# dayae1204/WeCLIP-ViT-CoMer

Measured on AMD Instinct MI355X. Metric: images/sec (train fwd+bwd) ViT-B/16 512x512 VOC, higher is better.
Workload: dtype f16 MFMA operands / f32 accumulate, f32 residual+softmax+LN, PAR f32 arithmetic on 16-bit fixed-point affinities (precision=fast); 1 GPU; WeCLIP VOC full train step (the reference's model: frozen CLIP ViT-B/16 + adapters + decoder + GradCAM/affinity/PAR pseudo-labels), batch 16/GPU at 512x512, K=2 classes/image (BASELINE configs[2] without the ViT-CoMer inserts, for which the reference has no code); global_batch=16, parallelism=dp1

## Files before the change

### weclip-vit-comer_amd/csrc/attention.hip

```cpp
#include "common.h"
#include <stdlib.h>

typedef _Float16 f16x8 __attribute__((ext_vector_type(8)));
typedef _Float16 f16x4 __attribute__((ext_vector_type(4)));
typedef _Float16 f16x2 __attribute__((ext_vector_type(2)));
typedef float f32x16 __attribute__((ext_vector_type(16)));

#define NEG_BIG (-1.0e30f)

template <int DH, int NT>
__device__ __forceinline__ void attn_row_body(const __half* __restrict__ qkv, __half* __restrict__ out,
                                              float* __restrict__ out32, float* __restrict__ lse, int L, int H,
                                              int E, int q, int h, int b, float* lds) {
    constexpr int NCH = DH / 8;
    constexpr int NPT = NT / NCH;
    float* sc = lds;
    float* red = lds + ((L + 3) & ~3);
    float (*part)[DH] = reinterpret_cast<float (*)[DH]>(red + 16);
    const int tid = threadIdx.x;
    const long ldq = 3L * E;
    const __half* base = qkv + (long)b * L * ldq + (long)h * DH;
    f16x8 qv[NCH];
#pragma unroll
    for (int c = 0; c < NCH; ++c) qv[c] = *reinterpret_cast<const f16x8*>(base + (long)q * ldq + c * 8);
    float mx = NEG_BIG;
    for (int key = tid; key < L; key += NT) {
        const __half* kr = base + E + (long)key * ldq;
        float s = 0.f;
#pragma unroll
        for (int c = 0; c < NCH; ++c) {
            const f16x8 kv = *reinterpret_cast<const f16x8*>(kr + c * 8);
#pragma unroll
            for (int j = 0; j < 8; ++j) s = fmaf((float)qv[c][j], (float)kv[j], s);
        }
        sc[key] = s;
        mx = fmaxf(mx, s);
    }
    mx = block_max(mx, red);
    float sum = 0.f;
    for (int key = tid; key < L; key += NT) {
        const float pr = __builtin_amdgcn_exp2f(sc[key] - mx);
        sum += pr;
        sc[key] = (float)(_Float16)pr;
    }
    sum = block_sum(sum, red);
    const int ch = tid % NCH, pt = tid / NCH;
    float o[8];
#pragma unroll
    for (int j = 0; j < 8; ++j) o[j] = 0.f;
    const __half* vcol = base + 2 * E + ch * 8;
    int key = pt;
    for (; key + 3 * NPT < L; key += 4 * NPT) {
        f16x8 v[4];
#pragma unroll
        for (int u = 0; u < 4; ++u) v[u] = *reinterpret_cast<const f16x8*>(vcol + (long)(key + u * NPT) * ldq);
#pragma unroll
        for (int u = 0; u < 4; ++u) {
            const float pr = sc[key + u * NPT];
#pragma unroll
            for (int j = 0; j < 8; ++j) o[j] = fmaf(pr, (float)v[u][j], o[j]);
        }
    }
    for (; key < L; key += NPT) {
        const f16x8 v = *reinterpret_cast<const f16x8*>(vcol + (long)key * ldq);
        const float pr = sc[key];
#pragma unroll
        for (int j = 0; j < 8; ++j) o[j] = fmaf(pr, (float)v[j], o[j]);
    }
#pragma unroll
    for (int j = 0; j < 8; ++j) part[pt][ch * 8 + j] = o[j];
    __syncthreads();
    if (tid < DH) {
        float v = 0.f;
        for (int k = 0; k < NPT; ++k) v += part[k][tid];
        v /= sum;
        const long oi = ((long)b * L + q) * E + (long)h * DH + tid;
        out[oi] = __float2half(v);
        if (out32) out32[oi] = v;
        if (tid == 0) lse[((long)b * H + h) * L + q] = mx + log2f(sum);
    }
}

#define ATT_EDGE_MAX 8
template <int DH, int NW>
__global__ __launch_bounds__(NW * 64, 4) void attn_fwd_kernel(const __half* __restrict__ qkv,
                                                        __half* __restrict__ out,
                                                        float* __restrict__ out32,
                                                        float* __restrict__ lse, int L, int H,
                                                        int E, int q_origin, int nqb, int Bn, int k_origin) {
    constexpr int NT = NW * 64;
    constexpr int KS = DH / 16;
    constexpr int DT = DH / 32;
    constexpr int KROW = DH * 2 + 16;
    constexpr int VROW = DH * 2;
    constexpr int KBUF = 64 * KROW, VBUF = 64 * VROW;
    constexpr int KCH = DH / 8;
    constexpr int TCH = 64 * KCH;
    constexpr int NKC = (TCH + NT - 1) / NT;
    constexpr int NVC = NKC;
    extern __shared__ __attribute__((aligned(16))) char smem[];

    const int tid = threadIdx.x, lane = tid & 63, wave = tid >> 6;
    const int hh = lane >> 5, l31 = lane & 31;
    const int per_img = nqb * H;
    const int main_blocks = per_img * ((Bn + 7) / 8 * 8);
    if ((int)blockIdx.x >= main_blocks) {
        const int e = blockIdx.x - main_blocks;
        const int hb = e / q_origin;
        attn_row_body<DH, NT>(qkv, out, out32, lse, L, H, E, e - hb * q_origin, hb % H, hb / H, reinterpret_cast<float*>(smem));
        return;
    }
    const int slot = blockIdx.x >> 3;
    const int b = (slot / per_img) * 8 + (blockIdx.x & 7);
    if (b >= Bn) return;
    const int rem = slot - (slot / per_img) * per_img;
    const int h = rem / nqb, qb = rem - h * nqb;
    const int qrow = q_origin + qb * (NW * 32) + wave * 32 + l31;
    const int qr = qrow < L ? qrow : L - 1;
    const long ldq = 3L * E;
    const __half* base = qkv + (long)b * L * ldq + (long)h * DH;

    f16x8 qf[KS];
#pragma unroll
    for (int s = 0; s < KS; ++s)
        qf[s] = *reinterpret_cast<const f16x8*>(base + (long)qr * ldq + 16 * s + 8 * hh);

    u32x4 rk[NKC], rv[NVC];
#define VSWZ(key_) (DH == 64 ? ((((key_) >> 1) & 1) << 2) : 0)
    int vaddr[2];
    {
        const int gi = (lane >> 4) & 1, q4 = (lane >> 2) & 3, p4 = lane & 3;
#pragma unroll
        for (int r = 0; r < 2; ++r) {
            const int key = 8 * r + 4 * hh + q4;
            vaddr[r] = key * VROW + (((2 * gi + (p4 >> 1)) ^ VSWZ(key)) << 4) + 8 * (p4 & 1);
        }
    }
    typedef short s16x4 __attribute__((__vector_size__(4 * sizeof(short))));
    typedef __attribute__((address_space(3))) s16x4* tr_ptr;
#undef GLOAD
#define GLOAD(t_) \
    { \
        const int t__ = (t_); \
        _Pragma("unroll") \
        for (int i = 0; i < NKC; ++i) { \
            const int c = (NKC * NT == TCH) ? tid + NT * i : (tid + NT * i) % TCH;    \
            int key = k_origin + t__ * 64 + c / KCH; \
            if (key > L - 1) key = L - 1; \
            rk[i] = *reinterpret_cast<const u32x4*>(base + E + (long)key * ldq + (c % KCH) * 8); \
        } \
        _Pragma("unroll") \
        for (int i = 0; i < NVC; ++i) { \
            const int c = (NKC * NT == TCH) ? tid + NT * i : (tid + NT * i) % TCH; \
            int key = k_origin + t__ * 64 + c / KCH; \
            if (key > L - 1) key = L - 1; \
            rv[i] = *reinterpret_cast<const u32x4*>(base + 2 * E + (long)key * ldq + (c % KCH) * 8); \
        } \
    }
#undef LSTORE
#define LSTORE(buf_) \
    { \
        const int buf__ = (buf_); \
        char* kb = smem + buf__ * (KBUF + VBUF); \
        char* vb = kb + KBUF; \
        _Pragma("unroll") \
        for (int i = 0; i < NKC; ++i) { \
            const int c = tid + NT * i; \
            if (c < TCH) *reinterpret_cast<u32x4*>(kb + (c / KCH) * KROW + (c % KCH) * 16) = rk[i]; \
        } \
        _Pragma("unroll") \
        for (int i = 0; i < NVC; ++i) { \
            const int c = tid + NT * i; \
            const int key__ = c / KCH; \
            if (c < TCH) *reinterpret_cast<u32x4*>(vb + key__ * VROW + (((c % KCH) ^ VSWZ(key__)) << 4)) = rv[i]; \
        } \
    }

    f32x16 o[DT];
#pragma unroll
    for (int d = 0; d < DT; ++d)
#pragma unroll
        for (int r = 0; r < 16; ++r) o[d][r] = 0.f;
    float m = NEG_BIG, lsum = 0.f;

    const int nt = (L - k_origin + 63) / 64;
    GLOAD(0);
    LSTORE(0);
    __syncthreads();
    for (int t = 0; t < nt; ++t) {
        const int buf = t & 1;
        if (t + 1 < nt) GLOAD(t + 1);
        const char* kb = smem + buf * (KBUF + VBUF);
        const char* vb = kb + KBUF;
        f32x16 s[2];
#pragma unroll
        for (int r = 0; r < 16; ++r) { s[0][r] = 0.f; s[1][r] = 0.f; }
#pragma unroll
        for (int ks = 0; ks < KS; ++ks) {
            const f16x8 a0 = *reinterpret_cast<const f16x8*>(kb + l31 * KROW + ks * 32 + hh * 16);
            const f16x8 a1 = *reinterpret_cast<const f16x8*>(kb + (32 + l31) * KROW + ks * 32 + hh * 16);
            s[0] = __builtin_amdgcn_mfma_f32_32x32x16_f16(a0, qf[ks], s[0], 0, 0, 0);
            s[1] = __builtin_amdgcn_mfma_f32_32x32x16_f16(a1, qf[ks], s[1], 0, 0, 0);
        }
        if (t == nt - 1) {
#pragma unroll
            for (int ti = 0; ti < 2; ++ti)
#pragma unroll
                for (int r = 0; r < 16; ++r) {
                    const int key = k_origin + t * 64 + ti * 32 + (r & 3) + 8 * (r >> 2) + 4 * hh;
                    if (key >= L) s[ti][r] = NEG_BIG;
                }
        }
        float mx = s[0][0];
#pragma unroll
        for (int r = 1; r < 16; ++r) mx = fmaxf(mx, s[0][r]);
#pragma unroll
        for (int r = 0; r < 16; ++r) mx = fmaxf(mx, s[1][r]);
        mx = fmaxf(mx, __shfl_xor(mx, 32, 64));
        const float mn = fmaxf(m, mx);
        const float alpha = __builtin_amdgcn_exp2f(m - mn);
        m = mn;
        lsum *= alpha;
#pragma unroll
        for (int d = 0; d < DT; ++d) o[d] *= alpha;
        typedef float f32x2 __attribute__((ext_vector_type(2)));
        const f32x2 nm = {-m, -m};
        f32x2 ps2 = {0.f, 0.f};
#pragma unroll
        for (int ti = 0; ti < 2; ++ti)
#pragma unroll
            for (int r = 0; r < 16; r += 2) {
                f32x2 e = {s[ti][r], s[ti][r + 1]};
                e += nm;
                f32x2 p;
                p[0] = __builtin_amdgcn_exp2f(e[0]);
                p[1] = __builtin_amdgcn_exp2f(e[1]);
                s[ti][r] = p[0];
                s[ti][r + 1] = p[1];
                ps2 += p;
            }
        lsum += ps2[0] + ps2[1];
#pragma unroll
        for (int s2 = 0; s2 < 4; ++s2) {
            f16x8 pb;
#pragma unroll
            for (int j = 0; j < 8; ++j) pb[j] = (_Float16)s[s2 >> 1][(s2 & 1) * 8 + j];
#pragma unroll
            for (int d = 0; d < DT; ++d) {
                const char* vr = vb + s2 * 16 * VROW;
                const f16x8 va = __builtin_bit_cast(f16x8, __builtin_shufflevector(
                    __builtin_amdgcn_ds_read_tr16_b64_v4i16((tr_ptr)(vr + (vaddr[0] ^ (d << 6)))),
                    __builtin_amdgcn_ds_read_tr16_b64_v4i16((tr_ptr)(vr + (vaddr[1] ^ (d << 6)))), 0, 1, 2, 3, 4, 5, 6, 7));
                o[d] = __builtin_amdgcn_mfma_f32_32x32x16_f16(va, pb, o[d], 0, 0, 0);
            }
        }
        if (t + 1 < nt) LSTORE(buf ^ 1);
        __syncthreads();
    }
    if constexpr (NW == 8)
    for (int kx = 0; kx < k_origin; ++kx) {
        const __half* krow = base + E + (long)kx * ldq;
        float sdot = 0.f;
#pragma unroll
        for (int ks = 0; ks < KS; ++ks) {
            const f16x8 kv = *reinterpret_cast<const f16x8*>(krow + 16 * ks + 8 * hh);
#pragma unroll
            for (int j = 0; j < 8; ++j) sdot = fmaf((float)qf[ks][j], (float)kv[j], sdot);
        }
        sdot += __shfl_xor(sdot, 32, 64);
        const float mn = fmaxf(m, sdot);
        const float alpha = __builtin_amdgcn_exp2f(m - mn);
        const float pr = __builtin_amdgcn_exp2f(sdot - mn);
        m = mn;
        lsum = lsum * alpha + (hh == 0 ? pr : 0.f);
        const float p16 = (float)(_Float16)pr;
        const __half* vrow = base + 2 * E + (long)kx * ldq;
#pragma unroll
        for (int d = 0; d < DT; ++d)
#pragma unroll
            for (int g = 0; g < 4; ++g) {
                const f16x4 vv = *reinterpret_cast<const f16x4*>(vrow + d * 32 + 8 * g + 4 * hh);
#pragma unroll
                for (int k = 0; k < 4; ++k) o[d][g * 4 + k] = fmaf(p16, (float)vv[k], o[d][g * 4 + k] * alpha);
            }
    }
    const float ltot = lsum + __shfl_xor(lsum, 32, 64);
    const float inv = 1.0f / ltot;
#ifdef WC_NO_OSTAGE
    constexpr bool OSTAGE = false;
#else
    constexpr bool OSTAGE = NW == 8;
#endif
    if constexpr (OSTAGE) {
        constexpr int OPITCH = DH * 2 + 8;
        constexpr int CPR = DH / 8;
        char* stg = smem + wave * (32 * OPITCH);
    #pragma unroll
        for (int d = 0; d < DT; ++d)
    #pragma unroll
            for (int g = 0; g < 4; ++g) {
                __half hv[4];
    #pragma unroll
                for (int k = 0; k < 4; ++k) hv[k] = __float2half(o[d][g * 4 + k] * inv);
                *reinterpret_cast<uint2*>(stg + l31 * OPITCH + (d * 32 + 8 * g + 4 * hh) * 2) = *reinterpret_cast<uint2*>(hv);
            }
        asm volatile("s_waitcnt lgkmcnt(0)" ::: "memory");
        __builtin_amdgcn_wave_barrier();
        const int qw0 = q_origin + qb * (NW * 32) + wave * 32;
    #pragma unroll
        for (int i = 0; i < 32 * CPR / 64; ++i) {
            const int r = i * (64 / CPR) + lane / CPR, ch = lane % CPR;
            if (qw0 + r < L) {
                const uint2 lo2 = *reinterpret_cast<const uint2*>(stg + r * OPITCH + ch * 16);
                const uint2 hi2 = *reinterpret_cast<const uint2*>(stg + r * OPITCH + ch * 16 + 8);
                u32x4 v = {lo2.x, lo2.y, hi2.x, hi2.y};
                *reinterpret_cast<u32x4*>(out + ((long)b * L + qw0 + r) * E + (long)h * DH + ch * 8) = v;
            }
        }
    } else if (qrow < L) {
        __half* orow = out + ((long)b * L + qrow) * E + (long)h * DH;
#pragma unroll
        for (int d = 0; d < DT; ++d)
#pragma unroll
            for (int g = 0; g < 4; ++g) {
                __half hv[4];
#pragma unroll
                for (int k = 0; k < 4; ++k) hv[k] = __float2half(o[d][g * 4 + k] * inv);
                *reinterpret_cast<uint2*>(orow + d * 32 + 8 * g + 4 * hh) = *reinterpret_cast<uint2*>(hv);
            }
    }
    if (qrow < L) {
        if (out32) {
#pragma unroll
            for (int d = 0; d < DT; ++d)
#pragma unroll
                for (int g = 0; g < 4; ++g)
                    *reinterpret_cast<float4*>(out32 + ((long)b * L + qrow) * E + (long)h * DH + d * 32 + 8 * g + 4 * hh) =
                        make_float4(o[d][g * 4] * inv, o[d][g * 4 + 1] * inv, o[d][g * 4 + 2] * inv, o[d][g * 4 + 3] * inv);
        }
        if (hh == 0) lse[((long)b * H + h) * L + qrow] = m + log2f(ltot);
    }
}

template <int DH, int R>
__global__ __launch_bounds__(256, 2) void attn_mean_kernel(const __half* __restrict__ qkv,
                                                         const float* __restrict__ lse,
                                                         float* __restrict__ mean, int L, int H, int E, int origin,
                                                         int nt, int Bn) {
    constexpr int KS = DH / 16;
    constexpr int ROW = DH * 2 + 16;
    constexpr int TB = 128 * ROW;
    constexpr int CH = DH / 8;
    constexpr int NC = 128 * CH / 256;
    extern __shared__ __attribute__((aligned(16))) char smem[];
    constexpr int EDGE = 2 * TB + 512;
    constexpr int BUF = EDGE + (R > 0 ? 2 * R * DH * 2 + 32 : 0);

    const int tid = threadIdx.x, lane = tid & 63, wave = tid >> 6;
    const int hh = lane >> 5, l31 = lane & 31;
    const int wr = wave >> 1, wc = wave & 1;
    const int slot = blockIdx.x >> 3;
    const int b = (slot / (nt * nt)) * 8 + (blockIdx.x & 7);
    if (b >= Bn) return;
    const int rem = slot - (slot / (nt * nt)) * (nt * nt);
    const int k0 = origin + (rem % nt) * 128, q0 = origin + (rem / nt) * 128;
    const long ldq = 3L * E;
    const __half* base = qkv + (long)b * L * ldq;

    const bool edge_wg = R > 0 && (q0 == origin || k0 == origin);
    const bool edge_row = R > 0 && q0 == origin && tid < 128;
    const bool edge_col = R > 0 && k0 == origin && tid >= 128;
    const int e_which = tid / (origin * CH > 0 ? origin * CH : 1);
    const int e_rem = tid - e_which * origin * CH;
    const __half* e_src = base + (long)(e_rem / CH) * ldq + (e_which ? E : 0) + (e_rem % CH) * 8;
    const int e_dst = EDGE + (e_which * R * CH + e_rem) * 16;
    u32x4 rq[NC], rk[NC], re = {0u, 0u, 0u, 0u};
    float rl = 0.f;
#undef GLOAD
#define GLOAD(h_) \
    { \
        const int h__ = (h_); \
        _Pragma("unroll") \
        for (int i = 0; i < NC; ++i) { \
            const int c = tid + 256 * i; \
            int qr = q0 + c / CH, kr = k0 + c / CH; \
            if (qr > L - 1) qr = L - 1; \
            if (kr > L - 1) kr = L - 1; \
            rq[i] = *reinterpret_cast<const u32x4*>(base + (long)qr * ldq + h__ * DH + (c % CH) * 8); \
            rk[i] = *reinterpret_cast<const u32x4*>(base + (long)kr * ldq + E + h__ * DH + (c % CH) * 8); \
        } \
        if (tid < 128) { \
            int qr = q0 + tid; \
            if (qr > L - 1) qr = L - 1; \
            rl = lse[((long)b * H + h__) * L + qr]; \
        } \
        if constexpr (R > 0) \
            if (edge_wg) { \
                if (e_which < 2) re = *reinterpret_cast<const u32x4*>(e_src + h__ * DH); \
                if (tid >= 128 && tid < 128 + origin) rl = lse[((long)b * H + h__) * L + tid - 128]; \
            } \
    }
#undef LSTORE
#define LSTORE(buf_) \
    { \
        const int buf__ = (buf_); \
        char* qb = smem + buf__ * BUF; \
        _Pragma("unroll") \
        for (int i = 0; i < NC; ++i) { \
            const int c = tid + 256 * i; \
            *reinterpret_cast<u32x4*>(qb + (c / CH) * ROW + (c % CH) * 16) = rq[i]; \
            *reinterpret_cast<u32x4*>(qb + TB + (c / CH) * ROW + (c % CH) * 16) = rk[i]; \
        } \
        if (tid < 128) reinterpret_cast<float*>(qb + 2 * TB)[tid] = rl; \
        if constexpr (R > 0) \
            if (edge_wg) { \
                if (e_which < 2) *reinterpret_cast<u32x4*>(qb + e_dst) = re; \
                if (tid >= 128 && tid < 128 + origin) reinterpret_cast<float*>(qb + EDGE + 2 * R * DH * 2)[tid - 128] = rl; \
            } \
    }

    f32x16 acc[2][2];
#pragma unroll
    for (int i = 0; i < 2; ++i)
#pragma unroll
        for (int j = 0; j < 2; ++j)
#pragma unroll
            for (int r = 0; r < 16; ++r) acc[i][j][r] = 0.f;
    f16x8 b_aug;
#pragma unroll
    for (int j = 0; j < 8; ++j) b_aug[j] = (_Float16)((hh == 0 && j < 2) ? 1.0f : 0.0f);
    float eacc[R > 0 ? R : 1];
#pragma unroll
    for (int e = 0; e < (R > 0 ? R : 1); ++e) eacc[e] = 0.f;

    GLOAD(0);
    LSTORE(0);
    __syncthreads();
    for (int h = 0; h < H; ++h) {
        const int buf = h & 1;
        if (h + 1 < H) GLOAD(h + 1);
        const char* qb = smem + buf * BUF;
        const float* ls = reinterpret_cast<const float*>(qb + 2 * TB);
        f16x8 a_aug[2];
#pragma unroll
        for (int mi = 0; mi < 2; ++mi) {
            const float nl = -ls[wr * 64 + mi * 32 + l31];
            const _Float16 hi = (_Float16)nl;
            const _Float16 lo = (_Float16)(nl - (float)hi);
#pragma unroll
            for (int j = 0; j < 8; ++j) a_aug[mi][j] = (_Float16)0.0f;
            if (hh == 0) { a_aug[mi][0] = hi; a_aug[mi][1] = lo; }
        }
        f32x16 s[2][2];
        {
            f32x16 zero;
#pragma unroll
            for (int r = 0; r < 16; ++r) zero[r] = 0.f;
            s[0][0] = __builtin_amdgcn_mfma_f32_32x32x16_f16(a_aug[0], b_aug, zero, 0, 0, 0);
            s[0][1] = __builtin_amdgcn_mfma_f32_32x32x16_f16(a_aug[0], b_aug, zero, 0, 0, 0);
            s[1][0] = __builtin_amdgcn_mfma_f32_32x32x16_f16(a_aug[1], b_aug, zero, 0, 0, 0);
            s[1][1] = __builtin_amdgcn_mfma_f32_32x32x16_f16(a_aug[1], b_aug, zero, 0, 0, 0);
        }
        const char* As = qb + (wr * 64 + l31) * ROW + hh * 16;
        const char* Bs = qb + TB + (wc * 64 + l31) * ROW + hh * 16;
#pragma unroll
        for (int ks = 0; ks < KS; ++ks) {
            const f16x8 a0 = *reinterpret_cast<const f16x8*>(As + ks * 32);
            const f16x8 a1 = *reinterpret_cast<const f16x8*>(As + 32 * ROW + ks * 32);
            const f16x8 b0 = *reinterpret_cast<const f16x8*>(Bs + ks * 32);
            const f16x8 b1 = *reinterpret_cast<const f16x8*>(Bs + 32 * ROW + ks * 32);
            s[0][0] = __builtin_amdgcn_mfma_f32_32x32x16_f16(a0, b0, s[0][0], 0, 0, 0);
            s[0][1] = __builtin_amdgcn_mfma_f32_32x32x16_f16(a0, b1, s[0][1], 0, 0, 0);
            s[1][0] = __builtin_amdgcn_mfma_f32_32x32x16_f16(a1, b0, s[1][0], 0, 0, 0);
            s[1][1] = __builtin_amdgcn_mfma_f32_32x32x16_f16(a1, b1, s[1][1], 0, 0, 0);
        }
#pragma unroll
        for (int mi = 0; mi < 2; ++mi)
#pragma unroll
            for (int ni = 0; ni < 2; ++ni)
#pragma unroll
                for (int r = 0; r < 16; ++r) acc[mi][ni][r] += __builtin_amdgcn_exp2f(s[mi][ni][r]);
        if constexpr (R > 0)
        if (edge_row || edge_col) {
            const int t = tid & 127;
            const char* own = qb + (edge_row ? TB : 0) + t * ROW;
            const char* oth = qb + EDGE + (edge_row ? 0 : R * DH * 2);
            float sd[R];
#pragma unroll
            for (int e = 0; e < R; ++e) sd[e] = 0.f;
#pragma unroll
            for (int c = 0; c < CH; ++c) {
                const f16x8 ov = *reinterpret_cast<const f16x8*>(own + c * 16);
#pragma unroll
                for (int e = 0; e < R; ++e)
                    if (R == 1 || e < origin) {
                        const f16x8 xv = *reinterpret_cast<const f16x8*>(oth + e * DH * 2 + c * 16);
#pragma unroll
                        for (int j = 0; j < 4; ++j)
                            sd[e] = __builtin_amdgcn_fdot2(f16x2{xv[2 * j], xv[2 * j + 1]}, f16x2{ov[2 * j], ov[2 * j + 1]}, sd[e], false);
                    }
            }
            const float own_lse = ls[t];
            const float* els = reinterpret_cast<const float*>(qb + EDGE + 2 * R * DH * 2);
#pragma unroll
            for (int e = 0; e < R; ++e)
                if (R == 1 || e < origin) eacc[e] += __builtin_amdgcn_exp2f(sd[e] - (edge_row ? els[e] : own_lse));
        }
        if (h + 1 < H) LSTORE(buf ^ 1);
        __syncthreads();
    }
    const float invh = 1.0f / H;
    float* mb = mean + (long)b * L * L;
#pragma unroll
    for (int mi = 0; mi < 2; ++mi)
#pragma unroll
        for (int ni = 0; ni < 2; ++ni) {
            const int key = k0 + wc * 64 + ni * 32 + l31;
            if (key >= L) continue;
#pragma unroll
            for (int r = 0; r < 16; ++r) {
                const int q = q0 + wr * 64 + mi * 32 + (r & 3) + 8 * (r >> 2) + 4 * hh;
                if (q < L) mb[(long)q * L + key] = acc[mi][ni][r] * invh;
            }
        }
    if constexpr (R > 0)
    if (edge_row || edge_col) {
        const int t = tid & 127;
#pragma unroll
        for (int e = 0; e < R; ++e)
            if (R == 1 || e < origin) {
                if (edge_row) { if (k0 + t < L) mb[(long)e * L + k0 + t] = eacc[e] * invh; }
                else if (q0 + t < L) mb[(long)(q0 + t) * L + e] = eacc[e] * invh;
            }
    }
    if (R > 0 && q0 == origin && k0 == origin && tid < origin * origin) {
        const int qe = tid / origin, ke = tid - qe * origin;
        float a = 0.f;
        for (int h = 0; h < H; ++h) {
            const __half* qr = base + (long)qe * ldq + h * DH;
            const __half* kr = base + (long)ke * ldq + E + h * DH;
            float sd = 0.f;
#pragma unroll
            for (int c = 0; c < CH; ++c) {
                const f16x8 xv = *reinterpret_cast<const f16x8*>(qr + c * 8);
                const f16x8 kv = *reinterpret_cast<const f16x8*>(kr + c * 8);
#pragma unroll
                for (int j = 0; j < 8; ++j) sd = fmaf((float)xv[j], (float)kv[j], sd);
            }
            a += __builtin_amdgcn_exp2f(sd - lse[((long)b * H + h) * L + qe]);
        }
        mb[(long)qe * L + ke] = a * invh;
    }
}

static int attn_origin(int L) {
    const int r = L % 128;
    return (L >= 128 && r > 0 && r <= ATT_EDGE_MAX) ? r : 0;
}

extern "C" int wc_attn_fwd(const void* qkv, void* out, float* out32, float* lse, int B, int L, int H, int DH,
                           void* stream) {
    const int E = H * DH;
    WC_CHECK_ARG(qkv && out && lse && B > 0 && L > 0 && H > 0, "wc_attn_fwd: bad argument");
    WC_CHECK_ARG(DH == 64 || DH == 32, "wc_attn_fwd: head dim must be 32 or 64 (got %d)", DH);
    WC_CHECK_ARG(((uintptr_t)qkv | (uintptr_t)out | (uintptr_t)out32) % 16 == 0, "wc_attn_fwd: operands must be 16-byte aligned");
    WC_CHECK_ARG(E % 8 == 0 && B <= 65535 && H <= 65535 && (long)wc_cdiv(L, 128) * H * (B + 7) < (1L << 30),
                 "wc_attn_fwd: bad shape");
    const size_t lds = DH == 64 ? 2 * (64 * (64 * 2 + 16) + 64 * 128) : 2 * (64 * (32 * 2 + 16) + 64 * 64);
    const int nw_env = 0;
    const int NWv = nw_env ? nw_env : ((DH == 64 && (long)wc_cdiv(L, 256) * H * B >= 512) ? 8 : 4);
    const int nthr = NWv * 64;
    int r = attn_origin(L);
    if (r && ((size_t)L + 4 + 16 + (nthr / (DH / 8)) * DH) * 4 > lds) r = 0;
    const int kr = (NWv == 8 && L >= 64 && L % 64 > 0 && L % 64 <= ATT_EDGE_MAX) ? L % 64 : 0;
    const int nqb = wc_cdiv(L - r, NWv * 32);
    dim3 grid((unsigned)(nqb * H * ((B + 7) / 8 * 8) + r * H * B));
    hipStream_t st = (hipStream_t)stream;
    const int pr = wc_prof_begin(stream);
    if (DH == 64 && NWv == 8)
        hipLaunchKernelGGL((attn_fwd_kernel<64, 8>), grid, dim3(512), lds, st, (const __half*)qkv, (__half*)out, out32, lse, L, H,
                           E, r, nqb, B, kr);
    else if (DH == 64)
        hipLaunchKernelGGL((attn_fwd_kernel<64, 4>), grid, dim3(256), lds, st, (const __half*)qkv, (__half*)out, out32, lse, L, H,
                           E, r, nqb, B, kr);
    else
        hipLaunchKernelGGL((attn_fwd_kernel<32, 4>), grid, dim3(256), lds, st, (const __half*)qkv, (__half*)out, out32, lse, L, H,
                           E, r, nqb, B, kr);
    wc_prof_end(pr, DH == 64 ? (NWv == 8 ? "attn_fwd_kernel<64, 8>" : "attn_fwd_kernel<64, 4>") : "attn_fwd_kernel<32, 4>",
                4.0 * B * H * (double)L * L * DH, stream);
    WC_LAUNCH_CHECK("attn_fwd_kernel");
    return WC_OK;
}

extern "C" int wc_attn_mean(const void* qkv, const float* lse, float* mean, int B, int L, int H, int DH,
                            void* stream) {
    const int E = H * DH;
    WC_CHECK_ARG(qkv && lse && mean && B > 0 && L > 0 && H > 0, "wc_attn_mean: bad argument");
    WC_CHECK_ARG(DH == 64 || DH == 32, "wc_attn_mean: head dim must be 32 or 64 (got %d)", DH);
    WC_CHECK_ARG((uintptr_t)qkv % 16 == 0, "wc_attn_mean: qkv must be 16-byte aligned");
    const int r = attn_origin(L);
    const int nt = wc_cdiv(L - r, 128);
    dim3 grid((unsigned)(nt * nt * ((B + 7) / 8 * 8)));
    hipStream_t st = (hipStream_t)stream;
    const int rcap = r == 0 ? 0 : (r == 1 ? 1 : ATT_EDGE_MAX);
    const size_t lds = 2 * ((size_t)2 * 128 * (DH * 2 + 16) + 512 + (rcap ? 2 * rcap * DH * 2 + 32 : 0));
    static bool lds_attr_set = false;
    if (!lds_attr_set) {
#define WC_MEAN_ATTR(DH_, R_) \
    (hipFuncSetAttribute((const void*)attn_mean_kernel<DH_, R_>, hipFuncAttributeMaxDynamicSharedMemorySize, 80 * 1024) == hipSuccess)
        WC_CHECK_ARG(WC_MEAN_ATTR(64, 0) && WC_MEAN_ATTR(64, 1) && WC_MEAN_ATTR(64, ATT_EDGE_MAX) && WC_MEAN_ATTR(32, 0) &&
                     WC_MEAN_ATTR(32, 1) && WC_MEAN_ATTR(32, ATT_EDGE_MAX), "wc_attn_mean: cannot reserve 80 KiB of LDS");
#undef WC_MEAN_ATTR
        lds_attr_set = true;
    }
    const int pr = wc_prof_begin(stream);
#define WC_MEAN_LAUNCH(DH_, R_) \
    hipLaunchKernelGGL((attn_mean_kernel<DH_, R_>), grid, dim3(256), lds, st, (const __half*)qkv, lse, mean, L, H, E, r, nt, B)
    if (DH == 64) {
        if (r == 0) WC_MEAN_LAUNCH(64, 0); else if (r == 1) WC_MEAN_LAUNCH(64, 1); else WC_MEAN_LAUNCH(64, ATT_EDGE_MAX);
    } else {
        if (r == 0) WC_MEAN_LAUNCH(32, 0); else if (r == 1) WC_MEAN_LAUNCH(32, 1); else WC_MEAN_LAUNCH(32, ATT_EDGE_MAX);
    }
#undef WC_MEAN_LAUNCH
    static const char* const mean_names[2][3] = {{"attn_mean_kernel<64, 0>", "attn_mean_kernel<64, 1>", "attn_mean_kernel<64, 8>"},
                                                 {"attn_mean_kernel<32, 0>", "attn_mean_kernel<32, 1>", "attn_mean_kernel<32, 8>"}};
    wc_prof_end(pr, mean_names[DH == 64 ? 0 : 1][r == 0 ? 0 : (r == 1 ? 1 : 2)], 2.0 * B * H * (double)L * L * DH, stream);
    WC_LAUNCH_CHECK("attn_mean_kernel");
    return WC_OK;
}
```

Before: 1321 images/sec.

## Add 256x256-tile MFMA head-mean attention kernel for head dim 64

After: 1307 images/sec. -1.1%, worse.

```diff
diff --git a/weclip-vit-comer_amd/csrc/attention.hip b/weclip-vit-comer_amd/csrc/attention.hip
--- a/weclip-vit-comer_amd/csrc/attention.hip
+++ b/weclip-vit-comer_amd/csrc/attention.hip
@@ -1,5 +1,6 @@
 #include "common.h"
 #include <stdlib.h>
+#include <type_traits>
 
 typedef _Float16 f16x8 __attribute__((ext_vector_type(8)));
 typedef _Float16 f16x4 __attribute__((ext_vector_type(4)));
@@ -81,6 +82,7 @@
     }
 }
 
+#define WC_MEAN_MI 4
 #define ATT_EDGE_MAX 8
 template <int DH, int NW>
 __global__ __launch_bounds__(NW * 64, 4) void attn_fwd_kernel(const __half* __restrict__ qkv,
@@ -542,6 +544,259 @@
             float sd = 0.f;
 #pragma unroll
             for (int c = 0; c < CH; ++c) {
+                const f16x8 xv = *reinterpret_cast<const f16x8*>(qr + c * 8);
+                const f16x8 kv = *reinterpret_cast<const f16x8*>(kr + c * 8);
+#pragma unroll
+                for (int j = 0; j < 8; ++j) sd = fmaf((float)xv[j], (float)kv[j], sd);
+            }
+            a += __builtin_amdgcn_exp2f(sd - lse[((long)b * H + h) * L + qe]);
+        }
+        mb[(long)qe * L + ke] = a * invh;
+    }
+}
+
+typedef float mf32x4 __attribute__((ext_vector_type(4)));
+template <int I, int N, class F>
+__device__ __forceinline__ void mean_static_for(F&& f) {
+    if constexpr (I < N) {
+        f(std::integral_constant<int, I>{});
+        mean_static_for<I + 1, N>(f);
+    }
+}
+
+template <int MI, int R>
+__global__ __launch_bounds__(512, 2) void attn_mean256_kernel(const __half* __restrict__ qkv,
+                                                            const float* __restrict__ lse,
+                                                            float* __restrict__ mean, int L, int H, int E, int origin,
+                                                            int nq, int nk, int Bn) {
+    constexpr int DH = 64;
+    constexpr int QT = MI * 64;
+    constexpr int TQ = QT * 128, TK = 256 * 128;
+    constexpr int NLS = TQ + TK;
+    constexpr int EDGE = NLS + QT * 4;
+    constexpr int STAGE = EDGE + (R > 0 ? 2 * R * 128 + 32 : 0);
+    extern __shared__ __attribute__((aligned(16))) char smem[];
+    typedef __attribute__((address_space(3))) void* lds_ptr;
+    typedef const __attribute__((address_space(1))) void* gbl_ptr;
+
+    const int tid = threadIdx.x, lane = tid & 63, wave = tid >> 6;
+    const int hh = lane >> 5, l31 = lane & 31;
+    const int wr = wave >> 2, wc = wave & 3;
+    const int slot = blockIdx.x >> 3;
+    const int ntile = nq * nk;
+    const int b = (slot / ntile) * 8 + (blockIdx.x & 7);
+    if (b >= Bn) return;
+    const int rem = slot - (slot / ntile) * ntile;
+    const int k0 = origin + (rem % nk) * 256, q0 = origin + (rem / nk) * QT;
+    const long ldq = 3L * E;
+    const __half* base = qkv + (long)b * L * ldq;
+
+    unsigned qoff[MI], koff[4];
+#pragma unroll
+    for (int i = 0; i < MI; ++i) {
+        const int row = wave * (QT / 8) + i * 8 + (lane >> 3);
+        const int c = (lane & 7) ^ ((row >> 1) & 7);
+        int gr = q0 + row;
+        if (gr > L - 1) gr = L - 1;
+        qoff[i] = (unsigned)gr * (unsigned)ldq + c * 8;
+    }
+#pragma unroll
+    for (int i = 0; i < 4; ++i) {
+        const int row = wave * 32 + i * 8 + (lane >> 3);
+        const int c = (lane & 7) ^ ((row >> 1) & 7);
+        int gr = k0 + row;
+        if (gr > L - 1) gr = L - 1;
+        koff[i] = (unsigned)gr * (unsigned)ldq + E + c * 8;
+    }
+    int lrow = (tid < QT ? q0 + tid : tid - QT);
+    if (lrow > L - 1) lrow = L - 1;
+    const bool l_tile = tid < QT, l_edge = R > 0 && tid >= QT && tid < QT + origin;
+
+    const bool edge_wg = R > 0 && (q0 == origin || k0 == origin);
+    const bool edge_row = R > 0 && q0 == origin && tid < 256;
+    const bool edge_col = R > 0 && k0 == origin && tid >= 256 && tid < 256 + QT;
+    const int e_which = tid / (origin * 8 > 0 ? origin * 8 : 1);
+    const int e_rem = tid - e_which * origin * 8;
+    const __half* e_src = base + (long)(e_rem / 8) * ldq + (e_which ? E : 0) + (e_rem % 8) * 8;
+    const int e_dst = EDGE + (e_which * R * 8 + e_rem) * 16;
+    u32x4 re = {0u, 0u, 0u, 0u};
+    float rl = 0.f;
+#undef GLOAD
+#define GLOAD(h_, buf_) \
+    { \
+        const __half* hb__ = base + (h_) * DH; \
+        char* dq__ = smem + (buf_) * STAGE + wave * (TQ / 8); \
+        char* dk__ = smem + (buf_) * STAGE + TQ + wave * 4096; \
+        _Pragma("unroll") \
+        for (int i = 0; i < MI; ++i) \
+            __builtin_amdgcn_global_load_lds((gbl_ptr)(hb__ + qoff[i]), (lds_ptr)(dq__ + i * 1024), 16, 0, 0); \
+        _Pragma("unroll") \
+        for (int i = 0; i < 4; ++i) \
+            __builtin_amdgcn_global_load_lds((gbl_ptr)(hb__ + koff[i]), (lds_ptr)(dk__ + i * 1024), 16, 0, 0); \
+        rl = lse[((long)b * H + (h_)) * L + lrow]; \
+        if constexpr (R > 0) \
+            if (edge_wg && e_which < 2) re = *reinterpret_cast<const u32x4*>(e_src + (h_) * DH); \
+    }
+#undef LSTORE
+#define LSTORE(buf_) \
+    { \
+        char* sb__ = smem + (buf_) * STAGE; \
+        if (l_tile) reinterpret_cast<float*>(sb__ + NLS)[tid] = -rl; \
+        if constexpr (R > 0) \
+            if (edge_wg) { \
+                if (e_which < 2) *reinterpret_cast<u32x4*>(sb__ + e_dst) = re; \
+                if (l_edge) reinterpret_cast<float*>(sb__ + EDGE + 2 * R * 128)[tid - QT] = -rl; \
+            } \
+    }
+
+    f32x16 acc[MI][2];
+#pragma unroll
+    for (int i = 0; i < MI; ++i)
+#pragma unroll
+        for (int j = 0; j < 2; ++j)
+#pragma unroll
+            for (int r = 0; r < 16; ++r) acc[i][j][r] = 0.f;
+    float eacc[R > 0 ? R : 1];
+#pragma unroll
+    for (int e = 0; e < (R > 0 ? R : 1); ++e) eacc[e] = 0.f;
+
+    const unsigned lbase = (unsigned)(size_t)(lds_ptr)smem;
+    unsigned xo[4];
+#pragma unroll
+    for (int ks = 0; ks < 4; ++ks) xo[ks] = (unsigned)(l31 * 128 + (((2 * ks + hh) ^ ((l31 >> 1) & 7)) << 4));
+    const unsigned a_off = (unsigned)(wr * (QT / 2) * 128), b_off = (unsigned)(TQ + wc * 64 * 128);
+    const unsigned c_off = (unsigned)(NLS + (wr * (QT / 2) + 4 * hh) * 4);
+
+    GLOAD(0, 0);
+    LSTORE(0);
+    __syncthreads();
+    for (int h = 0; h < H; ++h) {
+        const int buf = h & 1;
+        if (h + 1 < H) GLOAD(h + 1, buf ^ 1);
+        const unsigned sbase = lbase + (unsigned)(buf * STAGE);
+        f16x8 bf[2][4];
+#pragma unroll
+        for (int ks = 0; ks < 4; ++ks) {
+            const unsigned pb = sbase + b_off + xo[ks];
+            asm volatile("ds_read_b128 %0, %1" : "=v"(bf[0][ks]) : "v"(pb));
+            asm volatile("ds_read_b128 %0, %1 offset:4096" : "=v"(bf[1][ks]) : "v"(pb));
+        }
+        mean_static_for<0, MI>([&](auto mi_c) {
+            constexpr int mi = decltype(mi_c)::value;
+            f16x8 af[4];
+            mf32x4 c4[4];
+#pragma unroll
+            for (int ks = 0; ks < 4; ++ks)
+                asm volatile("ds_read_b128 %0, %1 offset:%2" : "=v"(af[ks]) : "v"(sbase + a_off + xo[ks]), "n"(mi * 32 * 128));
+            const unsigned pc = sbase + c_off;
+            asm volatile("ds_read_b128 %0, %1 offset:%2" : "=v"(c4[0]) : "v"(pc), "n"(mi * 128));
+            asm volatile("ds_read_b128 %0, %1 offset:%2" : "=v"(c4[1]) : "v"(pc), "n"(mi * 128 + 32));
+            asm volatile("ds_read_b128 %0, %1 offset:%2" : "=v"(c4[2]) : "v"(pc), "n"(mi * 128 + 64));
+            asm volatile("ds_read_b128 %0, %1 offset:%2" : "=v"(c4[3]) : "v"(pc), "n"(mi * 128 + 96));
+            if constexpr (mi == 0)
+                asm volatile("s_waitcnt lgkmcnt(0)"
+                             : "+v"(bf[0][0]), "+v"(bf[0][1]), "+v"(bf[0][2]), "+v"(bf[0][3]), "+v"(bf[1][0]), "+v"(bf[1][1]),
+                               "+v"(bf[1][2]), "+v"(bf[1][3]), "+v"(af[0]), "+v"(af[1]), "+v"(af[2]), "+v"(af[3]), "+v"(c4[0]),
+                               "+v"(c4[1]), "+v"(c4[2]), "+v"(c4[3]));
+            else
+                asm volatile("s_waitcnt lgkmcnt(0)"
+                             : "+v"(af[0]), "+v"(af[1]), "+v"(af[2]), "+v"(af[3]), "+v"(c4[0]), "+v"(c4[1]), "+v"(c4[2]), "+v"(c4[3]));
+            f32x16 c;
+#pragma unroll
+            for (int g = 0; g < 4; ++g) {
+                c[4 * g] = c4[g][0]; c[4 * g + 1] = c4[g][1]; c[4 * g + 2] = c4[g][2]; c[4 * g + 3] = c4[g][3];
+            }
+            f32x16 s0 = __builtin_amdgcn_mfma_f32_32x32x16_f16(af[0], bf[0][0], c, 0, 0, 0);
+            f32x16 s1 = __builtin_amdgcn_mfma_f32_32x32x16_f16(af[0], bf[1][0], c, 0, 0, 0);
+#pragma unroll
+            for (int ks = 1; ks < 4; ++ks) {
+                s0 = __builtin_amdgcn_mfma_f32_32x32x16_f16(af[ks], bf[0][ks], s0, 0, 0, 0);
+                s1 = __builtin_amdgcn_mfma_f32_32x32x16_f16(af[ks], bf[1][ks], s1, 0, 0, 0);
+            }
+#pragma unroll
+            for (int r = 0; r < 16; ++r) acc[mi][0][r] += __builtin_amdgcn_exp2f(s0[r]);
+#pragma unroll
+            for (int r = 0; r < 16; ++r) acc[mi][1][r] += __builtin_amdgcn_exp2f(s1[r]);
+            asm volatile("" : "+v"(acc[mi][0]), "+v"(acc[mi][1]));
+            __builtin_amdgcn_sched_barrier(0);
+        });
+        if constexpr (R > 0)
+        if (edge_row || edge_col) {
+            const int t = tid & 255;
+            const unsigned own = sbase + (unsigned)((edge_row ? TQ : 0) + t * 128);
+            const int oswz = (t >> 1) & 7;
+            const unsigned oth = sbase + (unsigned)(EDGE + (edge_row ? 0 : R * 128));
+            f16x8 ov[8];
+            float own_nl;
+#pragma unroll
+            for (int c = 0; c < 8; ++c) asm volatile("ds_read_b128 %0, %1" : "=v"(ov[c]) : "v"(own + (unsigned)((c ^ oswz) << 4)));
+            asm volatile("ds_read_b32 %0, %1" : "=v"(own_nl) : "v"(sbase + (unsigned)(NLS + (edge_row ? 0 : t) * 4)));
+            asm volatile("s_waitcnt lgkmcnt(0)"
+                         : "+v"(ov[0]), "+v"(ov[1]), "+v"(ov[2]), "+v"(ov[3]), "+v"(ov[4]), "+v"(ov[5]), "+v"(ov[6]), "+v"(ov[7]),
+                           "+v"(own_nl));
+#pragma unroll
+            for (int e = 0; e < R; ++e)
+                if (R == 1 || e < origin) {
+                    f16x8 xv[4];
+                    float enl;
+                    float sd = 0.f;
+#pragma unroll
+                    for (int hf = 0; hf < 2; ++hf) {
+#pragma unroll
+                        for (int c = 0; c < 4; ++c)
+                            asm volatile("ds_read_b128 %0, %1" : "=v"(xv[c]) : "v"(oth + (unsigned)(e * 128 + (hf * 4 + c) * 16)));
+                        if (hf == 0) {
+                            asm volatile("ds_read_b32 %0, %1" : "=v"(enl) : "v"(sbase + (unsigned)(EDGE + 2 * R * 128 + e * 4)));
+                            asm volatile("s_waitcnt lgkmcnt(0)" : "+v"(xv[0]), "+v"(xv[1]), "+v"(xv[2]), "+v"(xv[3]), "+v"(enl));
+                        } else {
+                            asm volatile("s_waitcnt lgkmcnt(0)" : "+v"(xv[0]), "+v"(xv[1]), "+v"(xv[2]), "+v"(xv[3]));
+                        }
+#pragma unroll
+                        for (int c = 0; c < 4; ++c)
+#pragma unroll
+                            for (int j = 0; j < 4; ++j)
+                                sd = __builtin_amdgcn_fdot2(f16x2{xv[c][2 * j], xv[c][2 * j + 1]},
+                                                            f16x2{ov[hf * 4 + c][2 * j], ov[hf * 4 + c][2 * j + 1]}, sd, false);
+                    }
+                    eacc[e] += __builtin_amdgcn_exp2f(sd + (edge_row ? enl : own_nl));
+                }
+        }
+        if (h + 1 < H) LSTORE(buf ^ 1);
+        __syncthreads();
+    }
+    const float invh = 1.0f / H;
+    float* mb = mean + (long)b * L * L;
+#pragma unroll
+    for (int mi = 0; mi < MI; ++mi)
+#pragma unroll
+        for (int ni = 0; ni < 2; ++ni) {
+            const int key = k0 + wc * 64 + ni * 32 + l31;
+            if (key >= L) continue;
+#pragma unroll
+            for (int r = 0; r < 16; ++r) {
+                const int q = q0 + wr * (QT / 2) + mi * 32 + (r & 3) + 8 * (r >> 2) + 4 * hh;
+                if (q < L) mb[(long)q * L + key] = acc[mi][ni][r] * invh;
+            }
+        }
+    if constexpr (R > 0)
+    if (edge_row || edge_col) {
+        const int t = tid & 255;
+#pragma unroll
+        for (int e = 0; e < R; ++e)
+            if (R == 1 || e < origin) {
+                if (edge_row) { if (k0 + t < L) mb[(long)e * L + k0 + t] = eacc[e] * invh; }
+                else if (q0 + t < L) mb[(long)(q0 + t) * L + e] = eacc[e] * invh;
+            }
+    }
+    if (R > 0 && q0 == origin && k0 == origin && tid < origin * origin) {
+        const int qe = tid / origin, ke = tid - qe * origin;
+        float a = 0.f;
+        for (int h = 0; h < H; ++h) {
+            const __half* qr = base + (long)qe * ldq + h * DH;
+            const __half* kr = base + (long)ke * ldq + E + h * DH;
+            float sd = 0.f;
+#pragma unroll
+            for (int c = 0; c < 8; ++c) {
                 const f16x8 xv = *reinterpret_cast<const f16x8*>(qr + c * 8);
                 const f16x8 kv = *reinterpret_cast<const f16x8*>(kr + c * 8);
 #pragma unroll
@@ -599,29 +854,40 @@
     WC_CHECK_ARG(DH == 64 || DH == 32, "wc_attn_mean: head dim must be 32 or 64 (got %d)", DH);
     WC_CHECK_ARG((uintptr_t)qkv % 16 == 0, "wc_attn_mean: qkv must be 16-byte aligned");
     const int r = attn_origin(L);
-    const int nt = wc_cdiv(L - r, 128);
-    dim3 grid((unsigned)(nt * nt * ((B + 7) / 8 * 8)));
     hipStream_t st = (hipStream_t)stream;
     const int rcap = r == 0 ? 0 : (r == 1 ? 1 : ATT_EDGE_MAX);
-    const size_t lds = 2 * ((size_t)2 * 128 * (DH * 2 + 16) + 512 + (rcap ? 2 * rcap * DH * 2 + 32 : 0));
     static bool lds_attr_set = false;
     if (!lds_attr_set) {
-#define WC_MEAN_ATTR(DH_, R_) \
-    (hipFuncSetAttribute((const void*)attn_mean_kernel<DH_, R_>, hipFuncAttributeMaxDynamicSharedMemorySize, 80 * 1024) == hipSuccess)
-        WC_CHECK_ARG(WC_MEAN_ATTR(64, 0) && WC_MEAN_ATTR(64, 1) && WC_MEAN_ATTR(64, ATT_EDGE_MAX) && WC_MEAN_ATTR(32, 0) &&
-                     WC_MEAN_ATTR(32, 1) && WC_MEAN_ATTR(32, ATT_EDGE_MAX), "wc_attn_mean: cannot reserve 80 KiB of LDS");
+#define WC_MEAN_ATTR(K_, KIB_) \
+    (hipFuncSetAttribute((const void*)K_, hipFuncAttributeMaxDynamicSharedMemorySize, KIB_ * 1024) == hipSuccess)
+        WC_CHECK_ARG(WC_MEAN_ATTR((attn_mean_kernel<32, 0>), 80) && WC_MEAN_ATTR((attn_mean_kernel<32, 1>), 80) &&
+                     WC_MEAN_ATTR((attn_mean_kernel<32, ATT_EDGE_MAX>), 80) &&
+                     WC_MEAN_ATTR((attn_mean256_kernel<WC_MEAN_MI, 0>), 144) && WC_MEAN_ATTR((attn_mean256_kernel<WC_MEAN_MI, 1>), 144) &&
+                     WC_MEAN_ATTR((attn_mean256_kernel<WC_MEAN_MI, ATT_EDGE_MAX>), 144),
+                     "wc_attn_mean: cannot reserve 80 KiB (head dim 32) / 144 KiB (head dim 64) of LDS");
 #undef WC_MEAN_ATTR
         lds_attr_set = true;
     }
     const int pr = wc_prof_begin(stream);
-#define WC_MEAN_LAUNCH(DH_, R_) \
-    hipLaunchKernelGGL((attn_mean_kernel<DH_, R_>), grid, dim3(256), lds, st, (const __half*)qkv, lse, mean, L, H, E, r, nt, B)
     if (DH == 64) {
-        if (r == 0) WC_MEAN_LAUNCH(64, 0); else if (r == 1) WC_MEAN_LAUNCH(64, 1); else WC_MEAN_LAUNCH(64, ATT_EDGE_MAX);
+        WC_CHECK_ARG((long)L * 3 * E < (1L << 32), "wc_attn_mean: image of %d x %d halves too large", L, 3 * E);
+        constexpr int QT = WC_MEAN_MI * 64;
+        const int nq = wc_cdiv(L - r, QT), nk = wc_cdiv(L - r, 256);
+        dim3 grid((unsigned)(nq * nk * ((B + 7) / 8 * 8)));
+        const size_t lds = 2 * ((size_t)(QT + 256) * 128 + QT * 4 + (rcap ? 2 * rcap * 128 + 32 : 0));
+#define WC_MEAN_LAUNCH(R_) \
+    hipLaunchKernelGGL((attn_mean256_kernel<WC_MEAN_MI, R_>), grid, dim3(512), lds, st, (const __half*)qkv, lse, mean, L, H, E, r, nq, nk, B)
+        if (r == 0) WC_MEAN_LAUNCH(0); else if (r == 1) WC_MEAN_LAUNCH(1); else WC_MEAN_LAUNCH(ATT_EDGE_MAX);
+#undef WC_MEAN_LAUNCH
     } else {
-        if (r == 0) WC_MEAN_LAUNCH(32, 0); else if (r == 1) WC_MEAN_LAUNCH(32, 1); else WC_MEAN_LAUNCH(32, ATT_EDGE_MAX);
-    }
+        const int nt = wc_cdiv(L - r, 128);
+        dim3 grid((unsigned)(nt * nt * ((B + 7) / 8 * 8)));
+        const size_t lds = 2 * ((size_t)2 * 128 * (DH * 2 + 16) + 512 + (rcap ? 2 * rcap * DH * 2 + 32 : 0));
+#define WC_MEAN_LAUNCH(R_) \
+    hipLaunchKernelGGL((attn_mean_kernel<32, R_>), grid, dim3(256), lds, st, (const __half*)qkv, lse, mean, L, H, E, r, nt, B)
+        if (r == 0) WC_MEAN_LAUNCH(0); else if (r == 1) WC_MEAN_LAUNCH(1); else WC_MEAN_LAUNCH(ATT_EDGE_MAX);
 #undef WC_MEAN_LAUNCH
+    }
     static const char* const mean_names[2][3] = {{"attn_mean_kernel<64, 0>", "attn_mean_kernel<64, 1>", "attn_mean_kernel<64, 8>"},
                                                  {"attn_mean_kernel<32, 0>", "attn_mean_kernel<32, 1>", "attn_mean_kernel<32, 8>"}};
     wc_prof_end(pr, mean_names[DH == 64 ? 0 : 1][r == 0 ? 0 : (r == 1 ? 1 : 2)], 2.0 * B * H * (double)L * L * DH, stream);
```
